# AlessioSam/LADiff

Hardware: AMD Instinct MI355X
Metric: motions/sec (196-frame, 50-step DDIM, bs128) (higher is better)
Workload: dtype f16x3+f32; 1 GPU; headline:ddim50_cfg7.5_b128_f196_c263_humanml3d; prompts_per_gpu=128, global_batch=128, frames=196, scheduler=ddim, denoising_steps=50, parallelism=dp1, loop=persistent pipeline kernel (16-row blocks x 86)

## Files before the change

### ladiff_amd/csrc/api.hip

```cpp
#include <algorithm>
#include <cstdlib>
#include <atomic>
#include <cstdio>
#include <cstdlib>
#include <cstring>
#include <vector>

#include "model.h"
#include "../../include/ladiff_hip_debug.h"

using namespace ladiff;

namespace {

inline hipStream_t S(ladiff_stream_t s) { return reinterpret_cast<hipStream_t>(s); }

template <class W>
bool load_weights(W& dst, const float* const* ptrs) {
    constexpr int n = sizeof(W) / sizeof(const float*);
    if (ptrs == nullptr) return false;
    for (int i = 0; i < n; ++i)
        if (ptrs[i] == nullptr) return false;
    std::memcpy(&dst, ptrs, sizeof(W));
    return true;
// ... 345 lines not shown
    g_handoff = tagged;
    return 0;
}

int ladiff_debug_set_mlp_variant(int v) {
#ifdef LADIFF_STAMPS
    LADIFF_CHECK_ARG((v >= 0 && v <= 3) || (v >= 11 && v <= 17) || (v >= 21 && v <= 26));
#else
    LADIFF_CHECK_ARG(v >= 0 && v <= 3);
#endif
    g_mlp_variant = v;
    return 0;
}

int ladiff_debug_set_decoder_fusion(int on) {
    LADIFF_CHECK_ARG(on >= 0 && on <= 126 && (on & 3) != 3 && (on & 48) != 48);
    g_dec_out_cross = (on & 64) ? 0 : 1;
    g_dec_fused_mlp = on & 3;
    g_dec_small_rows_path = (on & 4) ? 0 : 1;
    g_dec_final_split = (on & 8) ? 0 : 1;
    g_dec_fused_attn = (on & 16) ? 0 : (on & 32) ? 2 : 1;
    return 0;
}

int ladiff_debug_set_stage_plan(int v) {
    LADIFF_CHECK_ARG(v >= 0 && v <= 1);
    g_stage_plan = v;
    return 0;
}

int ladiff_debug_set_poll_pause(int mask, int len) {
// ... 445 lines not shown
    return 0;
}

int ladiff_vae_decode_graphed(void* graph, const float* const* w, const float* const* w_split, uint64_t weights_generation, const float* z,
                              const int32_t* lengths, const int32_t* counts, const int32_t* row_off, int total_rows, int B, int F, int T,
                              int C, float* feats, void* ws, size_t ws_bytes, ladiff_stream_t stream) {
    DecodeGraph* dg = reinterpret_cast<DecodeGraph*>(graph);
    DecoderW W, WS;
    LADIFF_CHECK_ARG(dg && load_weights(W, w) && z && lengths && feats && ws && B >= 0 && stream != nullptr);
    if (w_split != nullptr) LADIFF_CHECK_ARG(load_weights(WS, w_split));
    hipStream_t s = S(stream);
    const void* kp[7] = {z, lengths, counts, row_off, feats, ws, stream};
    const int ki[6] = {B, F, T, C, total_rows, w_split ? 1 : 0};
    uint64_t h = hash_ptrs(w, DEC_NPARAMS, 1469598103934665603ull);
    if (w_split) h = hash_ptrs(w_split, DEC_NPARAMS, h ^ 0x9e3779b97f4a7c15ull);
    h ^= (uint64_t)(g_dec_fused_mlp + 4 * g_dec_small_rows_path + 8 * g_dec_final_split + 16 * g_mlp_variant + 4096 * g_dec_fused_attn) * 0x100000001b3ull;
    const bool same = dg->exec && std::memcmp(kp, dg->key_ptrs, sizeof(kp)) == 0 && std::memcmp(ki, dg->key_ints, sizeof(ki)) == 0 &&
                      h == dg->key_hash && weights_generation == dg->key_gen &&
                      (dg->epoch == g_graph_epoch.load() || g_graph_epoch_rule.load() == 0);
    if (!same) {
        if (dg->exec) { LADIFF_HIP(hipStreamSynchronize(s)); (void)hipGraphExecDestroy(dg->exec); dg->exec = nullptr; }
        LADIFF_TRY(dec_mlp_prepare());
        LADIFF_TRY(dec_qkv_attn_prepare());
        LADIFF_TRY(dec_cross_prepare());
        hipGraph_t gr = nullptr;
        LADIFF_TRY(capture_stream(&dg->cap, &dg->cap_dev));
        const hipStream_t cs = dg->cap;
        LADIFF_HIP(hipStreamBeginCapture(cs, hipStreamCaptureModeThreadLocal));
        int rc = 0;
        if (row_off != nullptr) {
            rc = launch_zero_fill(feats, (size_t)B * F * C, cs);
        }
        if (rc == 0) rc = vae_decode(W, w_split ? &WS : nullptr, z, lengths, counts, row_off, total_rows, B, F, T, C, feats, (float*)ws,
                                     ws_bytes / sizeof(float), cs);
        const hipError_t ec = hipStreamEndCapture(cs, &gr);
        if (rc != 0) { if (gr) (void)hipGraphDestroy(gr); return rc; }
        LADIFF_HIP(ec);
        const hipError_t ei = hipGraphInstantiate(&dg->exec, gr, nullptr, nullptr, 0);
        ++g_graph_instantiations;
// ... 24 lines not shown
```

### ladiff_amd/csrc/attention.hip

```cpp
#include "kernels.h"

namespace ladiff {

constexpr int SA_FMAX = LADIFF_MAX_FRAMES;
constexpr int SA_NKT = SA_FMAX / 32;

struct AttnGeom { int nheads, ld, koff, voff, out_ld, causal; };

__global__ __launch_bounds__(256) void dec_self_attn_kernel(const float* __restrict__ qkv, const int32_t* __restrict__ lengths,
                                                            const uint32_t* __restrict__ keybits, float* __restrict__ out,
                                                            int B, int F, int split_out, const AttnGeom g,
                                                            const int32_t* __restrict__ row_off, int shared_qkv) {
    __shared__ __attribute__((aligned(16))) float Ks[SA_FMAX * DH];
    __shared__ __attribute__((aligned(16))) float Vs[SA_FMAX * DH];
    const int tid = threadIdx.x, lane = tid & 63, wave = tid >> 6;
    const int b = blockIdx.y / g.nheads, h = blockIdx.y % g.nheads;
    int len = F;
    uint32_t kb[SA_NKT + 1];
    if (keybits != nullptr) {
        len = 1;
#pragma unroll
        for (int i = 0; i < SA_NKT; ++i) {
            kb[i] = keybits[(size_t)b * 8 + i];
            if (kb[i]) len = 32 * i + 32 - __builtin_clz(kb[i]);
// ... 143 lines not shown
#pragma unroll
        for (int i = 0; i < NKT; ++i) {
            kb[i] = keybits[(size_t)b * 8 + i];
            if (kb[i]) len = 32 * i + 32 - __builtin_clz(kb[i]);
        }
        len = len > F ? F : len;
    } else {
        len = lengths != nullptr ? lengths[b] : F;
        len = len < 1 ? 1 : (len > F ? F : len);
#pragma unroll
        for (int i = 0; i < NKT; ++i) kb[i] = len >= 32 * i + 32 ? 0xFFFFFFFFu : (len > 32 * i ? (1u << (len - 32 * i)) - 1u : 0u);
    }
    const int nkt = (len + 31) >> 5;
    size_t row0 = (size_t)b * F;
    if (row_off != nullptr) { row0 = row_off[b]; F = row_off[b + 1] - row_off[b]; }
    const size_t base = (shared_qkv ? (size_t)0 : row0) * g.ld + h * DH;

    const int qt = wave;
    const int q = lane & 31, h2 = lane >> 5;
    const int qrow = qt * 32 + q;

    s16x8 qh[4], ql[4];
#pragma unroll
    for (int ks = 0; ks < 4; ++ks) {
        float v[8] = {0.f, 0.f, 0.f, 0.f, 0.f, 0.f, 0.f, 0.f};
        if (qrow < F) {
            const f32x4 a = ld4(qkv + base + (size_t)qrow * g.ld + 16 * ks + 8 * h2);
            const f32x4 c = ld4(qkv + base + (size_t)qrow * g.ld + 16 * ks + 8 * h2 + 4);
#pragma unroll
            for (int e = 0; e < 4; ++e) { v[e] = a[e] * (0.125f * 1.4426950408889634f); v[4 + e] = c[e] * (0.125f * 1.4426950408889634f); }
// ... 319 lines not shown
```

### ladiff_amd/csrc/dec_cross.hip

```cpp
#include <mutex>
#include "kernels.h"
#include "tile_mma.h"

namespace ladiff { extern unsigned long long* g_sys_stamps; }

namespace ladiff {

namespace {
constexpr int TM = LADIFF_MAX_LATENTS;
}

__global__ __launch_bounds__(256) void dec_cross_prep_kernel(const DecCrossPrepBatch pb, int B, int T, int tiles_per_wg) {
    const int h = blockIdx.y, layer = blockIdx.z, tid = threadIdx.x, lane = tid & 63, c16 = lane & 15, kq = lane >> 4;
    const int wave = __builtin_amdgcn_readfirstlane(tid >> 6);
    const float* __restrict__ kv = pb.kv[layer]; const float* __restrict__ wq = pb.wq[layer]; const float* __restrict__ bq = pb.bq[layer];
    const float* __restrict__ wo = pb.wo[layer]; float* __restrict__ gu = pb.gu[layer];
    float* __restrict__ cc = gu + (size_t)B * H * T * 2 * D;
    const int M = T * B, ntiles = (M + 15) / 16;
    float gq[4][16], uo[4][16], bqv[16];
#pragma unroll
    for (int t = 0; t < 4; ++t) {
        const int n = 64 * wave + 16 * t + c16;
#pragma unroll
        for (int s = 0; s < 16; ++s) gq[t][s] = wq[(size_t)(h * DH + 16 * kq + s) * D + n];
// ... 86 lines not shown
                const f32x4 u4 = ld4(up + 64 * k);
                acc[k][0] = fmaf(pj, u4[0], acc[k][0]); acc[k][1] = fmaf(pj, u4[1], acc[k][1]);
                acc[k][2] = fmaf(pj, u4[2], acc[k][2]); acc[k][3] = fmaf(pj, u4[3], acc[k][3]);
            }
        }
    }
}

template <int TT>
__global__ __launch_bounds__(256) void dec_cross_apply_kernel(const float* __restrict__ x, const float* __restrict__ gu,
                                                              const float* __restrict__ cc, const int32_t* __restrict__ counts,
                                                              const float* __restrict__ bo, const float* __restrict__ g2,
                                                              const float* __restrict__ b2, int F, int rows_per_wg,
                                                              float* __restrict__ y, float* __restrict__ ys,
                                                              const int32_t* __restrict__ row_off, const float* __restrict__ g1,
                                                              const float* __restrict__ b1) {
    extern __shared__ __attribute__((aligned(16))) float sm[];
    constexpr int T = TT, HT = H * TT;
    const int b = blockIdx.x, tid = threadIdx.x, lane = tid & 63, wave = tid >> 6;
    const float* src = gu + (size_t)b * HT * 2 * D;
    for (int u = tid; u < HT * 2 * D / 4; u += 256) st4(sm + 4 * u, ld4(src + 4 * u));
    float* cs = sm + (size_t)HT * 2 * D;
    if (tid < HT) cs[tid] = cc[(size_t)b * HT + tid];
    int nv = counts != nullptr ? counts[b] : T;
    nv = nv > T ? T : nv;
    __syncthreads();
    const int l16 = lane & 15, grp = lane >> 4, c0 = 4 * l16;
    f32x4 bo4[4], gg[4], bb[4];
#pragma unroll
    for (int k = 0; k < 4; ++k) { bo4[k] = ld4(bo + c0 + 64 * k); gg[k] = ld4(g2 + c0 + 64 * k); bb[k] = ld4(b2 + c0 + 64 * k); }
    size_t row0 = (size_t)b * F;
    if (row_off != nullptr) { row0 = row_off[b]; F = row_off[b + 1] - row_off[b]; }
    const int f0 = blockIdx.y * rows_per_wg;
    const int f1 = f0 + rows_per_wg < F ? f0 + rows_per_wg : F;
    for (int fb = f0; fb < f1; fb += 16) {
        const int f = fb + 4 * wave + grp;
        const bool live = f < f1;
        const size_t row = row0 + (live ? f : f1 - 1);
        f32x4 xv[4], acc[4];
#pragma unroll
        for (int k = 0; k < 4; ++k) xv[k] = ld4(x + row * D + c0 + 64 * k);
        if (g1 != nullptr) {
            float s1 = 0.f;
#pragma unroll
            for (int k = 0; k < 4; ++k) s1 += (xv[k][0] + xv[k][1]) + (xv[k][2] + xv[k][3]);
            const float mean1 = row16_sum(s1) * (1.f / 256.f);
            float q1 = 0.f;
#pragma unroll
            for (int k = 0; k < 4; ++k)
#pragma unroll
                for (int i = 0; i < 4; ++i) { const float dlt = xv[k][i] - mean1; q1 += dlt * dlt; }
            const float rstd1 = rsqrtf(row16_sum(q1) * (1.f / 256.f) + LN_EPS);
#pragma unroll
            for (int k = 0; k < 4; ++k) {
                const f32x4 ga = ld4(g1 + c0 + 64 * k), be = ld4(b1 + c0 + 64 * k);
#pragma unroll
// ... 348 lines not shown
}

int launch_decoder_cross_prep(const DecCrossPrepBatch& pb, int n, int B, int T, hipStream_t s) {
    if (B == 0 || n == 0) return 0;
    if (T < 1 || T > TM || n > DEC_PREP_MAX) return LADIFF_ERR_SHAPE;
    const int ntiles = (T * B + 15) / 16;
    int tpw = 1;
    while (tpw < 8 && (ntiles + 2 * tpw - 1) / (2 * tpw) * H * n >= 160) tpw *= 2;
    hipLaunchKernelGGL(dec_cross_prep_kernel, dim3((ntiles + tpw - 1) / tpw, H, n), dim3(256), 0, s, pb, B, T, tpw);
    LADIFF_LAUNCH_CHECK();
    return 0;
}

int launch_decoder_cross_apply(const float* x, const float* bo, const float* g2, const float* b2, const int32_t* counts, int B, int F,
                               int T, const float* gu_ws, float* y, float* ys, hipStream_t s, const int32_t* row_off, const float* g1,
                               const float* b1) {
    if (B == 0 || F == 0) return 0;
    if (T < 1 || T > TM) return LADIFF_ERR_SHAPE;
    const float* gu = gu_ws;
    const float* cc = gu_ws + (size_t)B * H * T * 2 * D;
    int chunks = (512 + B - 1) / B;
    if (chunks < 1) chunks = 1;
    if (chunks > (F + 3) / 4) chunks = (F + 3) / 4;
    const int rows_per_wg = ((F + chunks - 1) / chunks + 15) / 16 * 16;
    chunks = (F + rows_per_wg - 1) / rows_per_wg;
    const size_t lds = ((size_t)H * T * 2 * D + H * T) * sizeof(float);
    LADIFF_TRY(dec_cross_prepare());
#define LADIFF_DC_CASE(TT)                                                                                                   \
    case TT:                                                                                                                 \
        hipLaunchKernelGGL(dec_cross_apply_kernel<TT>, dim3(B, chunks), dim3(256), lds, s, x, gu, cc, counts, bo, g2, b2, F, \
                           rows_per_wg, y, ys, row_off, g1, b1);                                                                              \
        break;
    switch (T) {
        LADIFF_DC_CASE(1) LADIFF_DC_CASE(2) LADIFF_DC_CASE(3) LADIFF_DC_CASE(4)
        LADIFF_DC_CASE(5) LADIFF_DC_CASE(6) LADIFF_DC_CASE(7) LADIFF_DC_CASE(8)
        default: return LADIFF_ERR_SHAPE;
    }
#undef LADIFF_DC_CASE
    LADIFF_LAUNCH_CHECK();
    return 0;
}

int launch_decoder_out_cross(const float* att_s, const float* x0, const float* wo_s, const float* bo, const float* g1, const float* b1,
                             const float* bo_c, const float* g2, const float* b2, const int32_t* counts, int B, int F, int T,
                             const float* gu_ws, float* y, float* ys, hipStream_t s, const int32_t* row_off) {
    if (B == 0 || F == 0) return 0;
// ... 25 lines not shown
```

### ladiff_amd/csrc/decoder.hip

```cpp
#include "model.h"
#ifdef LADIFF_STAMPS
#include <cstdlib>
#endif

namespace ladiff {

#ifdef LADIFF_STAMPS
#define DEC_CUT() do { if (dec_cut >= 0 && ++dec_launched >= dec_cut) return 0; } while (0)
#else
#define DEC_CUT() do { } while (0)
#endif

constexpr int DEC_SMALL_ROWS = 4096;
std::atomic<int> g_dec_out_cross{1};
std::atomic<int> g_dec_fused_attn{1};
std::atomic<int> g_dec_final_split{1};
std::atomic<int> g_dec_small_rows_path{1};
std::atomic<int> g_dec_fused_mlp{1};

static GemmArgs lin(const float* A, int lda, const float* W, const float* bias, float* Y, int ldy, int M, int N, int K,
                    int act = ACT_NONE) {
    GemmArgs g;
    g.A = A; g.lda = lda; g.W = W; g.ldw = K; g.bias = bias; g.Y = Y; g.ldy = ldy; g.M = M; g.N = N; g.K = K; g.act = act;
    return g;
}

size_t dec_ws_floats(int B, size_t rows, int T) {
    return rows * (16 * D + 3 * D + D + FF) + (rows + 63) / 64 * 64 + (size_t)NL * ((size_t)T * B * 2 * D + dec_cross_ws_floats(B, T)) +
           (size_t)LADIFF_MAX_FRAMES * (2 * D + 3 * D);
}

int vae_decode(const DecoderW& w, const DecoderW* wsp, const float* z, const int32_t* lengths, const int32_t* counts,
               const int32_t* row_off, int R, int B, int F, int T, int C, float* feats, float* ws, size_t ws_floats, hipStream_t s) {
// ... 16 lines not shown
    for (int i = 0; i < 4; ++i) { P[i] = p; p += MD; }
    for (int i = 0; i < NSKIP; ++i) { SK[i] = p; p += MD; }
    for (int i = 0; i < 4; ++i) { Ps[i] = sp ? p : nullptr; p += MD; }
    for (int i = 0; i < NSKIP; ++i) { SKs[i] = sp ? p : nullptr; p += MD; }
    float* qkv = p; p += 3 * MD;
    float* att = p; p += MD;
    float* hid = p; p += (size_t)M * FF;
    float* kv = p; p += (size_t)NL * T * B * 2 * D;
    float* guws = p; p += (size_t)NL * dec_cross_ws_floats(B, T);
    int32_t* row_out = reinterpret_cast<int32_t*>(p); p += ((size_t)M + 63) / 64 * 64;
    float* pex = p; p += (size_t)LADIFF_MAX_FRAMES * D;
    float* pexs = p; p += (size_t)LADIFF_MAX_FRAMES * D;
    float* qkv0 = p;
    const size_t kv_l = (size_t)T * B * 2 * D, gu_l = dec_cross_ws_floats(B, T);

    {
        GemmArgs g[NL];
        DecCrossPrepBatch pb;
        for (int l = 0; l < NL; ++l) {
            const DecLayerW& L = w.layer[l];
            g[l] = lin(z, D, L.cross_attn.in_w + (size_t)D * D, L.cross_attn.in_b + D, kv + l * kv_l, 2 * D, T * B, 2 * D, D);
            pb.kv[l] = kv + l * kv_l; pb.wq[l] = L.cross_attn.in_w; pb.bq[l] = L.cross_attn.in_b; pb.wo[l] = L.cross_attn.out_w;
            pb.gu[l] = guws + l * gu_l;
        }
        LADIFF_TRY(launch_gemm_batch(g, NL, s)); DEC_CUT();
        LADIFF_TRY(launch_decoder_cross_prep(pb, NL, B, T, s)); DEC_CUT();
    }

    const bool small = sp && M < DEC_SMALL_ROWS && g_dec_small_rows_path;
    const bool fused_attn = sp && g_dec_fused_attn && (M >= DEC_SMALL_ROWS || g_dec_fused_attn == 2);
    auto krs = [&](const float* A, int K, const float* W, const float* bias, float* Y, float* Ys, int ldy, int N, int act,
                   const float* res, int rows) -> int {
        KrArgs g;
        g.A = A; g.lda = K; g.W = W; g.ldw = K; g.bias = bias; g.Y = Y; g.Ys = Ys; g.ldy = ldy; g.M = rows; g.N = N; g.K = K; g.act = act;
        g.res = res; g.ldres = D; g.split = 1;
        return launch_gemm_kr(g, s);
    };

    auto gemm_ln = [&](const float* A, int K, const float* W, const float* Wsp, const float* bias, const float* res,
                       const NormW& n1, const NormW* n2, float* dst, float* dsts) -> int {
        GemmArgs g = lin(A, K, sp ? Wsp : W, bias, dst, D, M, D, K);
        g.res = res; g.ldres = D;
        if (!sp) {
            g.ln_g = n1.g; g.ln_b = n1.b;
            if (n2) { g.ln2_g = n2->g; g.ln2_b = n2->b; }
            return launch_gemm(g, s);
        }
        g.split = 1;
        LADIFF_TRY(launch_gemm(g, s));
        if (n2)
            return launch_reduce_rows(dst, 1, M, nullptr, nullptr, RED_LN, n1.g, n1.b, nullptr, 0, nullptr, nullptr, 1, 1, 0,
                                      0, dst, dsts, s, nullptr, n2->g, n2->b);
        return launch_reduce_rows(dst, 1, M, nullptr, nullptr, RED_LN, n1.g, n1.b, nullptr, 0, nullptr, nullptr, 1, 1, 0, 0,
                                  dst, dsts, s);
    };

    if (ragged) { LADIFF_TRY(launch_broadcast_pe_ragged(w.query_pe, row_off, B, F, F, P[0], Ps[0], row_out, s)); DEC_CUT(); }
    else { LADIFF_TRY(launch_broadcast_pe(w.query_pe, B, F, P[0], Ps[0], s)); DEC_CUT(); }
    const float* cur = P[0]; const float* curs = Ps[0];
    for (int l = 0; l < NL; ++l) {
        const DecLayerW& L = w.layer[l];
        const DecLayerW& Ls = sp ? wsp->layer[l] : w.layer[l];
        const bool is_in = l < NSKIP, is_out = l > NSKIP, last = l == NL - 1;
        if (is_out) {
            const LinearW& sk = w.skip[l - NSKIP - 1];
            if (small) {
                RowLnArgs g;
                g.A = curs; g.lda = D; g.A2 = SKs[NL - 1 - l]; g.lda2 = D; g.K1 = D; g.W = wsp->skip[l - NSKIP - 1].w; g.ldw = 2 * D; g.bias = sk.b;
                g.Y = P[3]; g.Ys = Ps[3]; g.ldy = D; g.M = M; g.K = 2 * D;
                LADIFF_TRY(launch_gemm_rowln(g, s)); DEC_CUT();
            } else {
            GemmArgs g = lin(sp ? curs : cur, D, sp ? wsp->skip[l - NSKIP - 1].w : sk.w, sk.b, P[3], D, M, D, 2 * D);
            g.A2 = sp ? SKs[NL - 1 - l] : SK[NL - 1 - l]; g.lda2 = D; g.K1 = D;
// ... 7 lines not shown
            LADIFF_TRY(launch_broadcast_pe(w.query_pe, 1, F, pex, sp ? pexs : nullptr, s)); DEC_CUT();
            if (small) { LADIFF_TRY(krs(pexs, D, Ls.self_attn.in_w, L.self_attn.in_b, qkv0, nullptr, 3 * D, 3 * D, ACT_NONE, nullptr, F)); DEC_CUT(); }
            else {
            GemmArgs g = lin(sp ? pexs : pex, D, Ls.self_attn.in_w, L.self_attn.in_b, qkv0, 3 * D, F, 3 * D, D);
            g.split = sp ? 1 : 0;
            LADIFF_TRY(launch_gemm(g, s)); DEC_CUT();
            }
        } else if (fused_attn) {
        } else if (small) {
            LADIFF_TRY(krs(curs, D, Ls.self_attn.in_w, L.self_attn.in_b, qkv, nullptr, 3 * D, 3 * D, ACT_NONE, nullptr, M)); DEC_CUT();
        } else {
            GemmArgs g = lin(sp ? curs : cur, D, Ls.self_attn.in_w, L.self_attn.in_b, qkv, 3 * D, M, 3 * D, D);
            g.split = sp ? 1 : 0;
            LADIFF_TRY(launch_gemm(g, s)); DEC_CUT();
        }
        const float* qkv_l = shared ? qkv0 : qkv;
        if (fused_attn && !shared) { LADIFF_TRY(launch_dec_qkv_attn(curs, Ls.self_attn.in_w, L.self_attn.in_b, lengths, row_off, att, B, F, 1, s)); DEC_CUT(); }
        else if (sp) { LADIFF_TRY(launch_self_attention_split(qkv_l, lengths, nullptr, att, B, F, H, 0, 1, s, row_off, shared)); DEC_CUT(); }
        else { LADIFF_TRY(launch_decoder_self_attention(qkv_l, lengths, nullptr, att, B, F, 0, s, row_off, shared)); DEC_CUT(); }
        const NormW* n1_late = nullptr;
        if (sp && !small && g_dec_out_cross) {
            LADIFF_TRY(launch_decoder_out_cross(att, cur, Ls.self_attn.out_w, L.self_attn.out_b, L.norm1.g, L.norm1.b, L.cross_attn.out_b,
                                                L.norm2.g, L.norm2.b, counts, B, F, T, guws + l * gu_l, P[2], Ps[2], s, row_off)); DEC_CUT();
        } else {
        if (sp) {
            if (small) { LADIFF_TRY(krs(att, D, Ls.self_attn.out_w, L.self_attn.out_b, P[1], nullptr, D, D, ACT_NONE, cur, M)); DEC_CUT(); }
            else {
            GemmArgs g = lin(att, D, Ls.self_attn.out_w, L.self_attn.out_b, P[1], D, M, D, D);
            g.res = cur; g.ldres = D; g.split = 1;
            LADIFF_TRY(launch_gemm(g, s)); DEC_CUT();
            }
            n1_late = &L.norm1;
        } else {
            LADIFF_TRY(gemm_ln(att, D, L.self_attn.out_w, Ls.self_attn.out_w, L.self_attn.out_b, cur, L.norm1, nullptr, P[1], nullptr)); DEC_CUT();
        }
        LADIFF_TRY(launch_decoder_cross_apply(P[1], L.cross_attn.out_b, L.norm2.g, L.norm2.b, counts, B, F, T, guws + l * gu_l, P[2],
                                              Ps[2], s, row_off, n1_late ? n1_late->g : nullptr, n1_late ? n1_late->b : nullptr)); DEC_CUT();
        }
        float* dst = is_in ? SK[l] : P[0];
        float* dsts = is_in ? SKs[l] : Ps[0];
        if (sp && g_dec_fused_mlp && (M >= dec_mlp_min_rows() || g_dec_fused_mlp == 2)) {
            LADIFF_TRY(launch_dec_mlp(Ps[2], P[2], Ls.lin1.w, L.lin1.b, Ls.lin2.w, L.lin2.b, L.norm3.g, L.norm3.b,
                                      last ? w.norm.g : nullptr, last ? w.norm.b : nullptr, dst, dsts, M, s)); DEC_CUT();
        } else if (small) {
            LADIFF_TRY(krs(Ps[2], D, Ls.lin1.w, L.lin1.b, nullptr, hid, FF, FF, ACT_GELU, nullptr, M)); DEC_CUT();
            LADIFF_TRY(krs(hid, FF, Ls.lin2.w, nullptr, qkv, nullptr, D, D, ACT_NONE, nullptr, M)); DEC_CUT();
            LADIFF_TRY(launch_reduce_rows(qkv, 4, M, L.lin2.b, P[2], RED_LN, L.norm3.g, L.norm3.b, nullptr, 0, nullptr, nullptr, 1, 1, 0, 0,
                                          dst, dsts, s, nullptr, last ? w.norm.g : nullptr, last ? w.norm.b : nullptr));
        } else {
            GemmArgs g = lin(sp ? Ps[2] : P[2], D, Ls.lin1.w, L.lin1.b, sp ? nullptr : hid, FF, M, FF, D, ACT_GELU);
            g.split = sp ? 1 : 0; if (sp) g.Ys = hid;
            LADIFF_TRY(launch_gemm(g, s)); DEC_CUT();
// ... 22 lines not shown
```

### ladiff_amd/csrc/gemm_kr.h

```cpp
#pragma once
#include "common.h"

namespace ladiff {

struct KrArgs {
    const float* A = nullptr;  int lda = 0;
    const float* A2 = nullptr; int lda2 = 0;
    int K1 = 0;
    const float* W = nullptr;  int ldw = 0;
    const float* bias = nullptr;
    float* Y = nullptr;        int ldy = 0;
    float* Ys = nullptr;
    int split = 0;
    int M = 0, N = 0, K = 0;
    int act = ACT_NONE;
    const float* res = nullptr; int ldres = 0;
    unsigned long long* stamps = nullptr;
};

int launch_gemm_kr(const KrArgs& a, hipStream_t s);

struct RowLnArgs {
    const float* A = nullptr;  int lda = 0;
    const float* A2 = nullptr; int lda2 = 0; int K1 = 0;
    const float* W = nullptr;  int ldw = 0;
    const float* bias = nullptr;
    const float* res = nullptr; int ldres = 0;
    const float* ln_g = nullptr; const float* ln_b = nullptr;
    float* Y = nullptr; float* Ys = nullptr; int ldy = 0;
    int M = 0, K = 0;
};
int launch_gemm_rowln(const RowLnArgs& a, hipStream_t s);

struct CombineGemmArgs {
    const float* P = nullptr; size_t plane = 0; int S = 0;
    const float* bias2 = nullptr;
    const float* ln_g = nullptr; const float* ln_b = nullptr;
    const float* tab = nullptr; int tab_step_stride = 0; const int32_t* d_step = nullptr;
    const float* W = nullptr; int ldw = 0;
    const float* bias = nullptr;
    const float* res = nullptr; int ldres = 0;
    float* Y = nullptr; float* Ys = nullptr; int ldy = 0;
    int M = 0;
};
int launch_combine_gemm(const CombineGemmArgs& a, hipStream_t s);
// ... 3 lines not shown
```

### ladiff_amd/csrc/gemm_rowln.hip

```cpp
#include "gemm_kr.h"

namespace ladiff {

namespace {
template <int N> __device__ __forceinline__ void wait_vm() { asm volatile("s_waitcnt vmcnt(%0)" ::"n"(N) : "memory"); }
__device__ __forceinline__ void dma16(const float* g, float* l) {
    __builtin_amdgcn_global_load_lds(g, (__attribute__((address_space(3))) void*)l, 16, 0, 0);
}
}

__global__ __launch_bounds__(512) void gemm_rowln_kernel(const RowLnArgs p) {
    constexpr int BM = 16, BN = 256;
    constexpr int ROWS = BM + BN;
    constexpr int STAGE = ROWS * 64;
    constexpr int PCS = ROWS / 4;
    constexpr int PPW = PCS / 4;
    constexpr int RN = 4;
    constexpr int CLD = BN + 4;
    static_assert(2 * PPW <= 63, "vmcnt is 6 bits");

    __shared__ __attribute__((aligned(1024))) float lds[2 * STAGE];

    const int tid = threadIdx.x, lane = tid & 63;
    const int wave = __builtin_amdgcn_readfirstlane(tid >> 6);
    const int argM = pin_s(p.M), nk = pin_s(p.K) >> 6;
    const int row0 = blockIdx.x * BM;

    if (wave >= 4) {
        const int pw = wave - 4;
        const int rl = 4 * pw + (lane >> 4);
        const int kl = ((lane & 15) ^ rl) << 2;
        const float* const argA = pin_s(p.A); const float* const argW = pin_s(p.W);
        const int lda = pin_s(p.lda), ldw = pin_s(p.ldw);
        int gr = row0 + rl; gr = gr < argM ? gr : argM - 1;
        const float* const arow = argA + (size_t)gr * lda + kl;
        const int K1 = pin_s(p.K1);
        const float* const arow2 = p.A2 != nullptr ? p.A2 + (size_t)gr * p.lda2 + kl - K1 : arow;
        const float* const wrow = argW + (size_t)rl * ldw + kl;
        float* const lbase = lds + 4 * pw * 64;
        auto issue = [&](int kt) __attribute__((always_inline)) {
            float* const dst = lbase + (kt & 1) * STAGE;
// ... 13 lines not shown
        return;
    }

    float* const argY = pin_s(p.Y); float* const argYs = pin_s(p.Ys);
    const float* const argRes = pin_s(p.res);
    const int ldres = pin_s(p.ldres), ldy = pin_s(p.ldy);
    const int c = lane * 4;
    const f32x4 zero = {0.f, 0.f, 0.f, 0.f};
    const f32x4 bi = p.bias != nullptr ? ld4(p.bias + c) : zero;
    const bool ln = p.ln_g != nullptr;
    const f32x4 gg = ln ? ld4(p.ln_g + c) : zero, bb = ln ? ld4(p.ln_b + c) : zero;
    f32x4 rv[4];
#pragma unroll
    for (int e = 0; e < 4; ++e) {
        const int gr = row0 + 4 * wave + e;
        rv[e] = (argRes != nullptr && gr < argM) ? ld4g(argRes + (size_t)gr * ldres + c) : zero;
    }

    f32x4 acc[RN];
#pragma unroll
    for (int j = 0; j < RN; ++j) acc[j] = zero;
    const int frow = lane & 15, fk = lane >> 4;
    for (int kt = 0; kt < nk; ++kt) {
        const float* sa = lds + (kt & 1) * STAGE;
        const float* sb = sa + (BM + 64 * wave) * 64;
        __builtin_amdgcn_s_barrier();
        s16x8 ah[2], al[2], bh[2][RN], bl[2][RN];
#pragma unroll
        for (int g = 0; g < 2; ++g) {
            const int ch = 4 * g + fk, cl = 8 + 4 * g + fk;
            ah[g] = __builtin_bit_cast(s16x8, ld4(sa + frow * 64 + ((ch ^ frow) << 2)));
// ... 235 lines not shown
```

### ladiff_amd/csrc/kernels.h

```cpp
#pragma once
#include "common.h"
#include "noise_gen.h"

namespace ladiff {

enum RedMode : int { RED_PLAIN = 0, RED_LN = 1, RED_LN_ADD = 2, RED_LN_MOD = 3 };
int launch_reduce_rows(const float* P, int S, int M, const float* bias, const float* res, int mode, const float* g,
                       const float* b, const float* tab, int tab_step_stride, const int32_t* d_step,
                       const int32_t* counts, int Bs, int T, int pad_row, int b_off, float* out, float* outs, hipStream_t s,
                       const int32_t* d_base = nullptr, const float* g2 = nullptr, const float* b2 = nullptr);
int launch_split_rows(const float* x, float* y, int R, int K, hipStream_t s);
int launch_gather_rows(const float* src, const int32_t* index, int n_rows, int row_floats, float* dst, hipStream_t s);
int launch_split_range_stats(const float* const* xs, const int64_t* counts, int n, int64_t max_count, unsigned long long* stats,
                             hipStream_t s);
int launch_layernorm(const float* x, const float* g, const float* b, float* y, int M, hipStream_t s);
constexpr int DEC_PREP_MAX = 9;
struct DecCrossPrepBatch { const float* kv[DEC_PREP_MAX]; const float* wq[DEC_PREP_MAX]; const float* bq[DEC_PREP_MAX];
                           const float* wo[DEC_PREP_MAX]; float* gu[DEC_PREP_MAX]; };
constexpr int ROW_BATCH_MAX = 9;
struct RowBatch { const float* a[ROW_BATCH_MAX]; const float* g[ROW_BATCH_MAX]; const float* b[ROW_BATCH_MAX]; float* y[ROW_BATCH_MAX]; };
int launch_layernorm_batch(const RowBatch& rb, int n, int M, hipStream_t s);
int launch_ca_table_input_batch(const RowBatch& rb, int n_layers, int step_stride, int n, int B2, hipStream_t s, int split_out = 0);
int launch_ca_table_input(const float* nval, const float* beta, const float* mod, int step_stride, int n, int B2, float* u,
                          hipStream_t s);
int launch_add_pe(const float* sample, const float* pe, int Bs, int b_off, int b_n, int T, float* x, float* xs, hipStream_t s);
int launch_broadcast_pe(const float* pe, int B, int F, float* x, float* xs, hipStream_t s);
int launch_broadcast_pe_ragged(const float* pe, const int32_t* row_off, int B, int F, int F_out, float* x, float* xs, int32_t* row_out,
                               hipStream_t s);
int launch_relu(const float* x, float* y, size_t n, hipStream_t s);
int launch_pad_rows(const float* src, const float* srcb, float* dst, float* dstb, int C, int Np, hipStream_t s);
int launch_zero_fill(float* x, size_t n, hipStream_t s);
int launch_silu(const float* x, float* y, size_t n, hipStream_t s);
int launch_sinusoid(const int64_t* t, int n, float* out, hipStream_t s);
int launch_cfg_step(const float* eps, float* lat, const float* coef, const int32_t* d_step, const float* noise,
                    float g, int cfg, int B, int T, hipStream_t s);
int launch_advance(int32_t* d_step, hipStream_t s);
int launch_step_tail(float* x, float* xs, const float* ng, const float* nb, float* lat, const float* coef, int32_t* d_step,
                     const float* noise, const float* pe, float g, int cfg, int B, int T, hipStream_t s, const NoiseGen& gen = NoiseGen{0u, 0u, 0u, 0});
int launch_noise_fill(const NoiseGen& gen, int step0, int n, int B, int T, float* out, hipStream_t s);
int launch_init_latents(const float* noise, const int32_t* counts, float sigma, float* lat, int B, int T, hipStream_t s);
int launch_finalize_latents(const float* lat, const int32_t* counts, float* z, int B, int T, hipStream_t s, const unsigned* status = nullptr);

int launch_dec_qkv_attn(const float* xs, const float* w, const float* bias, const int32_t* lengths, const int32_t* row_off, float* out,
// ... 9 lines not shown
int launch_lca_kv(const float* key, const float* value, int B, int N, float* att, hipStream_t s);
int launch_lca_apply(const float* q, const float* att, const int32_t* counts, int Bs, int b_off, int b_n, int T, const float* mod,
                     int step_stride, int sample_stride, const int32_t* d_step, const float* g, const float* be, float* u,
                     hipStream_t s);
int launch_denoiser_self_attention_general(const float* qkv, const float* text_kv, int N, const float* tables, int kv_off,
                                           int step_stride, const int32_t* d_step, const int32_t* counts, int Bs, int b_off,
                                           int b_n, int T, float* out, hipStream_t s);

size_t dec_cross_ws_floats(int B, int T);
int launch_decoder_cross_prep(const DecCrossPrepBatch& pb, int n, int B, int T, hipStream_t s);
int launch_decoder_out_cross(const float* att_s, const float* x0, const float* wo_s, const float* bo, const float* g1, const float* b1,
                             const float* bo_c, const float* g2, const float* b2, const int32_t* counts, int B, int F, int T,
                             const float* gu_ws, float* y, float* ys, hipStream_t s, const int32_t* row_off);
int launch_decoder_cross_apply(const float* x, const float* bo, const float* g2, const float* b2, const int32_t* counts, int B, int F,
                               int T, const float* gu_ws, float* y, float* ys, hipStream_t s, const int32_t* row_off = nullptr,
                               const float* g1 = nullptr, const float* b1 = nullptr);

int launch_feats2joints(const float* feats, const float* mean, const float* stdv, int B, int F, int C, int J, float* joints,
                        hipStream_t s);

int launch_denoiser_self_attention(const float* qkv, const float* text_kv, const float* tables, int kv_off,
                                   int step_stride, const int32_t* d_step, const int32_t* counts, int Bs, int b_off,
                                   int b_n, int T, float* out, int split_out, hipStream_t s);
int launch_decoder_self_attention(const float* qkv, const int32_t* lengths, const uint32_t* keybits, float* out, int B, int F,
                                  int split_out, hipStream_t s, const int32_t* row_off = nullptr, int shared_qkv = 0);
int launch_self_attention(const float* qkv, const int32_t* lengths, const uint32_t* keybits, float* out, int B, int F, int nheads,
                          int causal, int split_out, hipStream_t s, const int32_t* row_off = nullptr);
int launch_self_attention_split(const float* qkv, const int32_t* lengths, const uint32_t* keybits, float* out, int B, int F,
                                 int nheads, int causal, int split_out, hipStream_t s, const int32_t* row_off = nullptr, int shared_qkv = 0);
int launch_decoder_cross_attention(const float* q, const float* kv, const int32_t* counts, float* out, int B, int F,
                                   int T, int split_out, hipStream_t s);
// ... 3 lines not shown
```

### ladiff_amd/csrc/model.h

```cpp
#pragma once
#include <atomic>
#include "gemm.h"
#include "gemm_kr.h"
#include "kernels.h"
#include "weights.h"

namespace ladiff {

constexpr int DEN_OFF_CA_MOD = 0;
constexpr int DEN_OFF_FFN_MOD = 2 * D;
constexpr int DEN_OFF_TIME_KV = 4 * D;
constexpr int DEN_LAYER_STRIDE = 6 * D;
constexpr int DEN_STEP_STRIDE = NL * DEN_LAYER_STRIDE;

size_t den_tables_floats(int n_steps);
size_t den_text_cache_floats(int B2, int n_steps, int ntxt = 1);
size_t den_text_ws_floats(int B2, int n_steps, int ntxt = 1);
size_t den_forward_ws_floats(int B2, int T);
int denoiser_time_tables(const DenoiserW& w, const float* sinus, int n, float* tables, float* ws, size_t ws_floats, hipStream_t s);
int denoiser_text_cache(const DenoiserW& w, const float* text, int B2, const float* tables, int n_steps, float* cache,
                        float* ws, size_t ws_floats, hipStream_t s, int ntxt = 1);
int denoiser_forward(const DenoiserW& w, const DenoiserW* w_split, const float* tables, const int32_t* d_step,
                     const float* cache, int n_steps, const float* sample, int Bs, int dup, int T, const int32_t* counts, float* eps, float* ws,
                     size_t ws_floats, hipStream_t s, int b_lo = 0, int b_n = -1, int loop_mode = 0, int ntxt = 1,
                     const int32_t* d_base = nullptr);
const float* den_cache_tkv(const float* cache, int B2, int ntxt);
const float* den_cache_ctab(const float* cache, int B2, int ntxt);
int denoiser_text_static(const DenoiserW& w, const float* text, int B2, float* cache, float* ws, size_t ws_floats, hipStream_t s);
int denoiser_ctab(const DenoiserW& w, const float* tables_lo, int n, float* cache, int B2, float* u, size_t u_floats, hipStream_t s,
                  const DenoiserW* w_split = nullptr);
int linear_cross_attention(const DenoiserW& w, int layer, const float* x, const float* xf, const float* emb, const int32_t* counts,
                           int B, int T, int N, float* out, float* ws, size_t ws_floats, hipStream_t s);
size_t linear_cross_attention_ws_floats(int B, int T, int N);
void den_loop_io(float* ws, int rows, float** x, float** xs);

extern std::atomic<int> g_dec_fused_mlp;
extern std::atomic<int> g_dec_small_rows_path;
extern std::atomic<int> g_dec_final_split;
extern std::atomic<int> g_dec_out_cross;
extern std::atomic<int> g_stage_plan;
extern std::atomic<int> g_poll_pause;
extern std::atomic<int> g_stage_delay;
extern std::atomic<int> g_pace;
extern std::atomic<int> g_look_ahead_from, g_small_upto;
extern std::atomic<int> g_dec_fused_attn;
extern std::atomic<int> g_mlp_variant;
int dec_mlp_prepare();
int dec_qkv_attn_prepare();
int dec_cross_prepare();
int dec_mlp_min_rows();
size_t dec_ws_floats(int B, size_t rows, int T);
int vae_decode(const DecoderW& w, const DecoderW* w_split, const float* z, const int32_t* lengths, const int32_t* counts,
               const int32_t* row_off, int R, int B, int F, int T, int C, float* feats, float* ws, size_t ws_floats, hipStream_t s);

int launch_dec_mlp(const float* xs, const float* x, const float* w1, const float* b1, const float* w2, const float* b2, const float* g3,
                   const float* be3, const float* g4, const float* be4, float* y, float* ys, int M, hipStream_t s);

size_t enc_ws_floats(int B, int F, int T, int C);
int vae_encode(const EncoderW& w, const EncoderW* w_split, const float* features, const int32_t* lengths,
               const int32_t* counts, const float* eps, int B, int F, int T, int C, float* mu, float* sd, float* latent, float* ws,
               size_t ws_floats, hipStream_t s);

#ifdef LADIFF_STAMPS
extern unsigned long long* g_sys_stamps;
// ... 42 lines not shown
```

### ladiff_amd/csrc/rowops.hip

```cpp
#include <algorithm>

#include "kernels.h"

namespace ladiff {

constexpr int ROWS_PER_BLOCK = 4;

__device__ __forceinline__ void row_stats(const f32x4 v, float& mean, float& rstd) {
    float s = wave_sum(v[0] + v[1] + v[2] + v[3]);
    mean = s * (1.f / 256.f);
    float q = 0.f;
#pragma unroll
    for (int i = 0; i < 4; ++i) { const float d = v[i] - mean; q += d * d; }
    q = wave_sum(q);
    rstd = rsqrtf(q * (1.f / 256.f) + LN_EPS);
}

__global__ __launch_bounds__(256) void layernorm_kernel(const float* __restrict__ x, const float* __restrict__ g,
                                                        const float* __restrict__ b, float* __restrict__ y, int M) {
    const int row = blockIdx.x * ROWS_PER_BLOCK + (threadIdx.x >> 6);
    const int c = (threadIdx.x & 63) * 4;
    if (row >= M) return;
    f32x4 v = ld4(x + (size_t)row * D + c);
    float mean, rstd;
// ... 189 lines not shown
    const int c = (threadIdx.x & 63) * 4;
    if (row >= M) return;
    const f32x4 v = ld4(pe + (size_t)(row % F) * D + c);
    st4(x + (size_t)row * D + c, v);
    if (xs != nullptr) store_split4(xs + (size_t)row * D, c, v);
}

__global__ __launch_bounds__(256) void broadcast_pe_ragged_kernel(const float* __restrict__ pe, const int32_t* __restrict__ row_off,
                                                                  int F, int F_out, float* __restrict__ x, float* __restrict__ xs,
                                                                  int32_t* __restrict__ row_out) {
    const int b = blockIdx.y, f = blockIdx.x * ROWS_PER_BLOCK + (threadIdx.x >> 6);
    const int c = (threadIdx.x & 63) * 4;
    const int r0 = row_off[b];
    if (f >= F || f >= row_off[b + 1] - r0) return;
    const size_t row = (size_t)r0 + f;
    const f32x4 v = ld4(pe + (size_t)f * D + c);
    st4(x + row * D + c, v);
    if (xs != nullptr) store_split4(xs + row * D, c, v);
    if (c == 0) row_out[row] = b * F_out + f;
}
int launch_broadcast_pe_ragged(const float* pe, const int32_t* row_off, int B, int F, int F_out, float* x, float* xs, int32_t* row_out,
                               hipStream_t s) {
    if (B == 0) return 0;
    hipLaunchKernelGGL(broadcast_pe_ragged_kernel, dim3((F + ROWS_PER_BLOCK - 1) / ROWS_PER_BLOCK, B), dim3(256), 0, s, pe, row_off, F,
                       F_out, x, xs, row_out);
    LADIFF_LAUNCH_CHECK();
    return 0;
}

int launch_broadcast_pe(const float* pe, int B, int F, float* x, float* xs, hipStream_t s) {
    const int M = B * F;
    hipLaunchKernelGGL(broadcast_pe_kernel, dim3((M + ROWS_PER_BLOCK - 1) / ROWS_PER_BLOCK), dim3(256), 0, s, pe, F, M, x, xs);
    LADIFF_LAUNCH_CHECK();
    return 0;
}

__global__ __launch_bounds__(256) void gather_rows_kernel(const float* __restrict__ src, const int32_t* __restrict__ index, int n_rows,
                                                          int row4, float* __restrict__ dst) {
    const int row = blockIdx.x * ROWS_PER_BLOCK + (threadIdx.x >> 6);
    if (row >= n_rows) return;
// ... 420 lines not shown
```

Baseline: 11390 motions/s.

## Dedupe decoder layer-0 self-attention by unique length and overlap cross prep on side stream

New measurement: 11400 motions/s, median of 2. About the same (+0.0%).

```diff
diff --git a/ladiff_amd/csrc/api.hip b/ladiff_amd/csrc/api.hip
--- a/ladiff_amd/csrc/api.hip
+++ b/ladiff_amd/csrc/api.hip
@@ -383,7 +383,8 @@
 }
 
 int ladiff_debug_set_decoder_fusion(int on) {
-    LADIFF_CHECK_ARG(on >= 0 && on <= 126 && (on & 3) != 3 && (on & 48) != 48);
+    LADIFF_CHECK_ARG(on >= 0 && on <= 254 && (on & 3) != 3 && (on & 48) != 48);
+    g_dec_layer0_table = (on & 128) ? 0 : 1;
     g_dec_out_cross = (on & 64) ? 0 : 1;
     g_dec_fused_mlp = on & 3;
     g_dec_small_rows_path = (on & 4) ? 0 : 1;
@@ -859,7 +860,8 @@
     const int ki[6] = {B, F, T, C, total_rows, w_split ? 1 : 0};
     uint64_t h = hash_ptrs(w, DEC_NPARAMS, 1469598103934665603ull);
     if (w_split) h = hash_ptrs(w_split, DEC_NPARAMS, h ^ 0x9e3779b97f4a7c15ull);
-    h ^= (uint64_t)(g_dec_fused_mlp + 4 * g_dec_small_rows_path + 8 * g_dec_final_split + 16 * g_mlp_variant + 4096 * g_dec_fused_attn) * 0x100000001b3ull;
+    h ^= (uint64_t)(g_dec_fused_mlp + 4 * g_dec_small_rows_path + 8 * g_dec_final_split + 16 * g_mlp_variant + 4096 * g_dec_fused_attn + 16384 * g_dec_out_cross +
+                    32768 * g_dec_layer0_table) * 0x100000001b3ull;
     const bool same = dg->exec && std::memcmp(kp, dg->key_ptrs, sizeof(kp)) == 0 && std::memcmp(ki, dg->key_ints, sizeof(ki)) == 0 &&
                       h == dg->key_hash && weights_generation == dg->key_gen &&
                       (dg->epoch == g_graph_epoch.load() || g_graph_epoch_rule.load() == 0);
@@ -868,6 +870,7 @@
         LADIFF_TRY(dec_mlp_prepare());
         LADIFF_TRY(dec_qkv_attn_prepare());
         LADIFF_TRY(dec_cross_prepare());
+        LADIFF_TRY(dec_front_prepare());
         hipGraph_t gr = nullptr;
         LADIFF_TRY(capture_stream(&dg->cap, &dg->cap_dev));
         const hipStream_t cs = dg->cap;
diff --git a/ladiff_amd/csrc/attention.hip b/ladiff_amd/csrc/attention.hip
--- a/ladiff_amd/csrc/attention.hip
+++ b/ladiff_amd/csrc/attention.hip
@@ -181,6 +181,7 @@
     const int nkt = (len + 31) >> 5;
     size_t row0 = (size_t)b * F;
     if (row_off != nullptr) { row0 = row_off[b]; F = row_off[b + 1] - row_off[b]; }
+    if (F <= 0) return;
     const size_t base = (shared_qkv ? (size_t)0 : row0) * g.ld + h * DH;
 
     const int qt = wave;
diff --git a/ladiff_amd/csrc/dec_cross.hip b/ladiff_amd/csrc/dec_cross.hip
--- a/ladiff_amd/csrc/dec_cross.hip
+++ b/ladiff_amd/csrc/dec_cross.hip
@@ -124,7 +124,8 @@
                                                               const float* __restrict__ b2, int F, int rows_per_wg,
                                                               float* __restrict__ y, float* __restrict__ ys,
                                                               const int32_t* __restrict__ row_off, const float* __restrict__ g1,
-                                                              const float* __restrict__ b1) {
+                                                              const float* __restrict__ b1, const int32_t* __restrict__ tab_off,
+                                                              const int32_t* __restrict__ len_idx) {
     extern __shared__ __attribute__((aligned(16))) float sm[];
     constexpr int T = TT, HT = H * TT;
     const int b = blockIdx.x, tid = threadIdx.x, lane = tid & 63, wave = tid >> 6;
@@ -143,13 +144,28 @@
     if (row_off != nullptr) { row0 = row_off[b]; F = row_off[b + 1] - row_off[b]; }
     const int f0 = blockIdx.y * rows_per_wg;
     const int f1 = f0 + rows_per_wg < F ? f0 + rows_per_wg : F;
+    size_t trow0 = 0;
+    int tlen = F;
+    if (tab_off != nullptr) { const int u = len_idx[b]; trow0 = tab_off[u]; tlen = tab_off[u + 1] - tab_off[u]; }
     for (int fb = f0; fb < f1; fb += 16) {
         const int f = fb + 4 * wave + grp;
         const bool live = f < f1;
         const size_t row = row0 + (live ? f : f1 - 1);
+        if (tab_off != nullptr && f >= tlen) {
+            if (live) {
+                const f32x4 z4 = {0.f, 0.f, 0.f, 0.f};
+#pragma unroll
+                for (int k = 0; k < 4; ++k) {
+                    st4(y + row * D + c0 + 64 * k, z4);
+                    if (ys != nullptr) store_split4(ys + row * D, c0 + 64 * k, z4);
+                }
+            }
+            continue;
+        }
+        const size_t xrow = tab_off != nullptr ? trow0 + f : row;
         f32x4 xv[4], acc[4];
 #pragma unroll
-        for (int k = 0; k < 4; ++k) xv[k] = ld4(x + row * D + c0 + 64 * k);
+        for (int k = 0; k < 4; ++k) xv[k] = ld4(x + xrow * D + c0 + 64 * k);
         if (g1 != nullptr) {
             float s1 = 0.f;
 #pragma unroll
@@ -528,7 +544,8 @@
 
 int launch_decoder_cross_apply(const float* x, const float* bo, const float* g2, const float* b2, const int32_t* counts, int B, int F,
                                int T, const float* gu_ws, float* y, float* ys, hipStream_t s, const int32_t* row_off, const float* g1,
-                               const float* b1) {
+                               const float* b1, const int32_t* tab_off, const int32_t* len_idx) {
+    if ((tab_off == nullptr) != (len_idx == nullptr)) return LADIFF_ERR_ARG;
     if (B == 0 || F == 0) return 0;
     if (T < 1 || T > TM) return LADIFF_ERR_SHAPE;
     const float* gu = gu_ws;
@@ -543,7 +560,7 @@
 #define LADIFF_DC_CASE(TT)                                                                                                   \
     case TT:                                                                                                                 \
         hipLaunchKernelGGL(dec_cross_apply_kernel<TT>, dim3(B, chunks), dim3(256), lds, s, x, gu, cc, counts, bo, g2, b2, F, \
-                           rows_per_wg, y, ys, row_off, g1, b1);                                                                              \
+                           rows_per_wg, y, ys, row_off, g1, b1, tab_off, len_idx);                                                                          \
         break;
     switch (T) {
         LADIFF_DC_CASE(1) LADIFF_DC_CASE(2) LADIFF_DC_CASE(3) LADIFF_DC_CASE(4)
diff --git a/ladiff_amd/csrc/decoder.hip b/ladiff_amd/csrc/decoder.hip
--- a/ladiff_amd/csrc/decoder.hip
+++ b/ladiff_amd/csrc/decoder.hip
@@ -1,4 +1,6 @@
 #include "model.h"
+#include <mutex>
+#include <vector>
 #ifdef LADIFF_STAMPS
 #include <cstdlib>
 #endif
@@ -17,6 +19,50 @@
 std::atomic<int> g_dec_final_split{1};
 std::atomic<int> g_dec_small_rows_path{1};
 std::atomic<int> g_dec_fused_mlp{1};
+
+std::atomic<int> g_dec_layer0_table{1};
+
+namespace {
+struct FrontSet { int dev; bool busy; hipStream_t side; hipEvent_t fork, join; };
+std::mutex g_front_mu;
+std::vector<FrontSet*> g_front_sets;
+FrontSet* front_acquire() {
+    int dev = 0;
+    if (hipGetDevice(&dev) != hipSuccess) return nullptr;
+    std::lock_guard<std::mutex> lock(g_front_mu);
+    for (FrontSet* f : g_front_sets) if (f->dev == dev && !f->busy) { f->busy = true; return f; }
+    FrontSet* f = new FrontSet{dev, true, nullptr, nullptr, nullptr};
+    if (hipStreamCreateWithFlags(&f->side, hipStreamNonBlocking) != hipSuccess ||
+        hipEventCreateWithFlags(&f->fork, hipEventDisableTiming) != hipSuccess ||
+        hipEventCreateWithFlags(&f->join, hipEventDisableTiming) != hipSuccess) {
+        if (f->fork) (void)hipEventDestroy(f->fork);
+        if (f->side) (void)hipStreamDestroy(f->side);
+        delete f;
+        return nullptr;
+    }
+    g_front_sets.push_back(f);
+    return f;
+}
+void front_release(FrontSet* f) { std::lock_guard<std::mutex> lock(g_front_mu); f->busy = false; }
+struct FrontHold {
+    FrontSet* f = nullptr;
+    hipStream_t s = nullptr;
+    bool forked = false;
+    int join() {
+        if (!forked) return 0;
+        forked = false;
+        return (int)hipStreamWaitEvent(s, f->join, 0);
+    }
+    ~FrontHold() { if (f) { (void)join(); front_release(f); } }
+};
+}
+
+int dec_front_prepare() {
+    FrontSet* f = front_acquire();
+    if (f == nullptr) return (int)hipErrorOutOfMemory;
+    front_release(f);
+    return 0;
+}
 
 static GemmArgs lin(const float* A, int lda, const float* W, const float* bias, float* Y, int ldy, int M, int N, int K,
                     int act = ACT_NONE) {
@@ -63,7 +109,20 @@
     float* qkv0 = p;
     const size_t kv_l = (size_t)T * B * 2 * D, gu_l = dec_cross_ws_floats(B, T);
 
+    const bool small = sp && M < DEC_SMALL_ROWS && g_dec_small_rows_path;
+    const int U = B < LADIFF_MAX_FRAMES ? B : LADIFF_MAX_FRAMES;
+    const bool l0tab = sp && g_dec_layer0_table && (size_t)2 * U + 1 + B + M <= 3 * MD;
+    FrontHold front;
+    if (l0tab && !small) {
+        front.f = front_acquire();
+        if (front.f == nullptr) return (int)hipErrorOutOfMemory;
+        front.s = s;
+        LADIFF_HIP(hipEventRecord(front.f->fork, s));
+        LADIFF_HIP(hipStreamWaitEvent(front.f->side, front.f->fork, 0));
+        front.forked = true;
+    }
     {
+        const hipStream_t zs = front.f ? front.f->side : s;
         GemmArgs g[NL];
         DecCrossPrepBatch pb;
         for (int l = 0; l < NL; ++l) {
@@ -72,11 +131,13 @@
             pb.kv[l] = kv + l * kv_l; pb.wq[l] = L.cross_attn.in_w; pb.bq[l] = L.cross_attn.in_b; pb.wo[l] = L.cross_attn.out_w;
             pb.gu[l] = guws + l * gu_l;
         }
-        LADIFF_TRY(launch_gemm_batch(g, NL, s)); DEC_CUT();
-        LADIFF_TRY(launch_decoder_cross_prep(pb, NL, B, T, s)); DEC_CUT();
-    }
-
-    const bool small = sp && M < DEC_SMALL_ROWS && g_dec_small_rows_path;
+        int rc = launch_gemm_batch(g, NL, zs);
+        if (rc == 0) rc = launch_decoder_cross_prep(pb, NL, B, T, zs);
+        if (front.f) { const hipError_t e = hipEventRecord(front.f->join, zs); if (rc == 0) rc = (int)e; }
+        if (rc != 0) return rc;
+        DEC_CUT(); DEC_CUT();
+    }
+
     const bool fused_attn = sp && g_dec_fused_attn && (M >= DEC_SMALL_ROWS || g_dec_fused_attn == 2);
     auto krs = [&](const float* A, int K, const float* W, const float* bias, float* Y, float* Ys, int ldy, int N, int act,
                    const float* res, int rows) -> int {
@@ -104,8 +165,14 @@
                                   dst, dsts, s);
     };
 
-    if (ragged) { LADIFF_TRY(launch_broadcast_pe_ragged(w.query_pe, row_off, B, F, F, P[0], Ps[0], row_out, s)); DEC_CUT(); }
-    else { LADIFF_TRY(launch_broadcast_pe(w.query_pe, B, F, P[0], Ps[0], s)); DEC_CUT(); }
+    if (ragged) { LADIFF_TRY(launch_broadcast_pe_ragged(w.query_pe, row_off, B, F, F, l0tab ? nullptr : P[0], l0tab ? nullptr : Ps[0], row_out, s)); DEC_CUT(); }
+    else if (!l0tab) { LADIFF_TRY(launch_broadcast_pe(w.query_pe, B, F, P[0], Ps[0], s)); DEC_CUT(); }
+    int32_t* tab_len = reinterpret_cast<int32_t*>(qkv);
+    int32_t* tab_off = tab_len + U;
+    int32_t* len_idx = tab_off + U + 1;
+    int32_t* tab_f = len_idx + B;
+    float* att_tab = att;
+    float* n1tab = hid;
     const float* cur = P[0]; const float* curs = Ps[0];
     for (int l = 0; l < NL; ++l) {
         const DecLayerW& L = w.layer[l];
@@ -143,6 +210,17 @@
             g.split = sp ? 1 : 0;
             LADIFF_TRY(launch_gemm(g, s)); DEC_CUT();
         }
+        if (shared && l0tab) {
+            LADIFF_TRY(launch_dec_len_table(lengths, row_off, B, F, U, tab_len, tab_off, len_idx, tab_f, s)); DEC_CUT();
+            LADIFF_TRY(launch_self_attention_split(qkv0, tab_len, nullptr, att_tab, U, F, H, 0, 1, s, tab_off, 1)); DEC_CUT();
+            RowLnArgs g;
+            g.A = att_tab; g.lda = D; g.K1 = D; g.W = Ls.self_attn.out_w; g.ldw = D; g.bias = L.self_attn.out_b; g.res = pex; g.ldres = D;
+            g.res_map = tab_f; g.ln_g = L.norm1.g; g.ln_b = L.norm1.b; g.Y = n1tab; g.ldy = D; g.M = M; g.K = D; g.d_M = tab_off + U;
+            LADIFF_TRY(launch_gemm_rowln(g, s)); DEC_CUT();
+            LADIFF_TRY(front.join());
+            LADIFF_TRY(launch_decoder_cross_apply(n1tab, L.cross_attn.out_b, L.norm2.g, L.norm2.b, counts, B, F, T, guws + l * gu_l, P[2],
+                                                  Ps[2], s, row_off, nullptr, nullptr, tab_off, len_idx)); DEC_CUT();
+        } else {
         const float* qkv_l = shared ? qkv0 : qkv;
         if (fused_attn && !shared) { LADIFF_TRY(launch_dec_qkv_attn(curs, Ls.self_attn.in_w, L.self_attn.in_b, lengths, row_off, att, B, F, 1, s)); DEC_CUT(); }
         else if (sp) { LADIFF_TRY(launch_self_attention_split(qkv_l, lengths, nullptr, att, B, F, H, 0, 1, s, row_off, shared)); DEC_CUT(); }
@@ -165,6 +243,7 @@
         }
         LADIFF_TRY(launch_decoder_cross_apply(P[1], L.cross_attn.out_b, L.norm2.g, L.norm2.b, counts, B, F, T, guws + l * gu_l, P[2],
                                               Ps[2], s, row_off, n1_late ? n1_late->g : nullptr, n1_late ? n1_late->b : nullptr)); DEC_CUT();
+        }
         }
         float* dst = is_in ? SK[l] : P[0];
         float* dsts = is_in ? SKs[l] : Ps[0];
diff --git a/ladiff_amd/csrc/gemm_kr.h b/ladiff_amd/csrc/gemm_kr.h
--- a/ladiff_amd/csrc/gemm_kr.h
+++ b/ladiff_amd/csrc/gemm_kr.h
@@ -29,6 +29,8 @@
     const float* ln_g = nullptr; const float* ln_b = nullptr;
     float* Y = nullptr; float* Ys = nullptr; int ldy = 0;
     int M = 0, K = 0;
+    const int32_t* d_M = nullptr;
+    const int32_t* res_map = nullptr;
 };
 int launch_gemm_rowln(const RowLnArgs& a, hipStream_t s);
 
diff --git a/ladiff_amd/csrc/gemm_rowln.hip b/ladiff_amd/csrc/gemm_rowln.hip
--- a/ladiff_amd/csrc/gemm_rowln.hip
+++ b/ladiff_amd/csrc/gemm_rowln.hip
@@ -23,8 +23,12 @@
 
     const int tid = threadIdx.x, lane = tid & 63;
     const int wave = __builtin_amdgcn_readfirstlane(tid >> 6);
-    const int argM = pin_s(p.M), nk = pin_s(p.K) >> 6;
+    const int nk = pin_s(p.K) >> 6;
     const int row0 = blockIdx.x * BM;
+    int argM_ = p.M;
+    if (p.d_M != nullptr) { const int m = __builtin_amdgcn_readfirstlane(*p.d_M); argM_ = m < argM_ ? m : argM_; }
+    const int argM = pin_s(argM_);
+    if (row0 >= argM) return;
 
     if (wave >= 4) {
         const int pw = wave - 4;
@@ -68,7 +72,7 @@
 #pragma unroll
     for (int e = 0; e < 4; ++e) {
         const int gr = row0 + 4 * wave + e;
-        rv[e] = (argRes != nullptr && gr < argM) ? ld4g(argRes + (size_t)gr * ldres + c) : zero;
+        rv[e] = (argRes != nullptr && gr < argM) ? ld4g(argRes + (size_t)(p.res_map != nullptr ? p.res_map[gr] : gr) * ldres + c) : zero;
     }
 
     f32x4 acc[RN];
diff --git a/ladiff_amd/csrc/kernels.h b/ladiff_amd/csrc/kernels.h
--- a/ladiff_amd/csrc/kernels.h
+++ b/ladiff_amd/csrc/kernels.h
@@ -27,6 +27,8 @@
 int launch_broadcast_pe(const float* pe, int B, int F, float* x, float* xs, hipStream_t s);
 int launch_broadcast_pe_ragged(const float* pe, const int32_t* row_off, int B, int F, int F_out, float* x, float* xs, int32_t* row_out,
                                hipStream_t s);
+int launch_dec_len_table(const int32_t* lengths, const int32_t* row_off, int B, int F, int U, int32_t* tab_len, int32_t* tab_off,
+                         int32_t* len_idx, int32_t* tab_f, hipStream_t s);
 int launch_relu(const float* x, float* y, size_t n, hipStream_t s);
 int launch_pad_rows(const float* src, const float* srcb, float* dst, float* dstb, int C, int Np, hipStream_t s);
 int launch_zero_fill(float* x, size_t n, hipStream_t s);
@@ -66,7 +68,8 @@
                              const float* gu_ws, float* y, float* ys, hipStream_t s, const int32_t* row_off);
 int launch_decoder_cross_apply(const float* x, const float* bo, const float* g2, const float* b2, const int32_t* counts, int B, int F,
                                int T, const float* gu_ws, float* y, float* ys, hipStream_t s, const int32_t* row_off = nullptr,
-                               const float* g1 = nullptr, const float* b1 = nullptr);
+                               const float* g1 = nullptr, const float* b1 = nullptr, const int32_t* tab_off = nullptr,
+                               const int32_t* len_idx = nullptr);
 
 int launch_feats2joints(const float* feats, const float* mean, const float* stdv, int B, int F, int C, int J, float* joints,
                         hipStream_t s);
diff --git a/ladiff_amd/csrc/model.h b/ladiff_amd/csrc/model.h
--- a/ladiff_amd/csrc/model.h
+++ b/ladiff_amd/csrc/model.h
@@ -38,6 +38,7 @@
 extern std::atomic<int> g_dec_small_rows_path;
 extern std::atomic<int> g_dec_final_split;
 extern std::atomic<int> g_dec_out_cross;
+extern std::atomic<int> g_dec_layer0_table;
 extern std::atomic<int> g_stage_plan;
 extern std::atomic<int> g_poll_pause;
 extern std::atomic<int> g_stage_delay;
@@ -48,6 +49,7 @@
 int dec_mlp_prepare();
 int dec_qkv_attn_prepare();
 int dec_cross_prepare();
+int dec_front_prepare();
 int dec_mlp_min_rows();
 size_t dec_ws_floats(int B, size_t rows, int T);
 int vae_decode(const DecoderW& w, const DecoderW* w_split, const float* z, const int32_t* lengths, const int32_t* counts,
diff --git a/ladiff_amd/csrc/rowops.hip b/ladiff_amd/csrc/rowops.hip
--- a/ladiff_amd/csrc/rowops.hip
+++ b/ladiff_amd/csrc/rowops.hip
@@ -227,9 +227,11 @@
     const int r0 = row_off[b];
     if (f >= F || f >= row_off[b + 1] - r0) return;
     const size_t row = (size_t)r0 + f;
-    const f32x4 v = ld4(pe + (size_t)f * D + c);
-    st4(x + row * D + c, v);
-    if (xs != nullptr) store_split4(xs + row * D, c, v);
+    if (x != nullptr) {
+        const f32x4 v = ld4(pe + (size_t)f * D + c);
+        st4(x + row * D + c, v);
+        if (xs != nullptr) store_split4(xs + row * D, c, v);
+    }
     if (c == 0) row_out[row] = b * F_out + f;
 }
 int launch_broadcast_pe_ragged(const float* pe, const int32_t* row_off, int B, int F, int F_out, float* x, float* xs, int32_t* row_out,
@@ -237,6 +239,49 @@
     if (B == 0) return 0;
     hipLaunchKernelGGL(broadcast_pe_ragged_kernel, dim3((F + ROWS_PER_BLOCK - 1) / ROWS_PER_BLOCK, B), dim3(256), 0, s, pe, row_off, F,
                        F_out, x, xs, row_out);
+    LADIFF_LAUNCH_CHECK();
+    return 0;
+}
+
+__global__ __launch_bounds__(256) void dec_len_table_kernel(const int32_t* __restrict__ lengths, const int32_t* __restrict__ row_off, int B,
+                                                            int F, int U, int32_t* __restrict__ tab_len, int32_t* __restrict__ tab_off,
+                                                            int32_t* __restrict__ len_idx, int32_t* __restrict__ tab_f) {
+    static_assert(LADIFF_MAX_FRAMES + 2 <= 256, "a thread per length, one more for the totals");
+    __shared__ int present[256], slot[256], offs[256];
+    __shared__ unsigned long long mask[4];
+    const int v = threadIdx.x;
+    auto length_of = [&](int b) {
+        int e = row_off != nullptr ? row_off[b + 1] - row_off[b] : (lengths[b] < 1 ? 1 : lengths[b]);
+        e = e > F ? F : e;
+        return e < 0 ? 0 : e;
+    };
+    present[v] = 0;
+    __syncthreads();
+    for (int b = v; b < B; b += 256) { const int e = length_of(b); if (e > 0) present[e] = 1; }
+    __syncthreads();
+    const unsigned long long mine = __ballot(present[v] != 0);
+    if ((v & 63) == 0) mask[v >> 6] = mine;
+    __syncthreads();
+    int rank = 0, off = 0;
+    for (int q = 0; q < 4; ++q) {
+        unsigned long long m = mask[q];
+        if (64 * q + 63 >= v) m &= v > 64 * q ? (1ull << (v - 64 * q)) - 1ull : 0ull;
+        while (m) { const int w = 64 * q + __builtin_ctzll(m); ++rank; off += w; m &= m - 1; }
+    }
+    slot[v] = rank; offs[v] = off;
+    if (v >= 1 && v <= F && present[v] && rank < U) { tab_len[rank] = v; tab_off[rank] = off; }
+    __syncthreads();
+    const int nu = slot[F + 1], total = offs[F + 1];
+    if (v >= nu && v < U) { tab_len[v] = 0; tab_off[v] = total; }
+    if (v == 0) tab_off[U] = total;
+    for (int b = v; b < B; b += 256) { const int e = length_of(b); len_idx[b] = e > 0 ? slot[e] : 0; }
+    for (int q = 0; q < 4; ++q)
+        for (unsigned long long m = mask[q]; m; m &= m - 1) { const int w = 64 * q + __builtin_ctzll(m); if (v < w) tab_f[offs[w] + v] = v; }
+}
+int launch_dec_len_table(const int32_t* lengths, const int32_t* row_off, int B, int F, int U, int32_t* tab_len, int32_t* tab_off,
+                         int32_t* len_idx, int32_t* tab_f, hipStream_t s) {
+    if (B < 1 || F < 1 || F > LADIFF_MAX_FRAMES || U < 1 || U > LADIFF_MAX_FRAMES) return LADIFF_ERR_SHAPE;
+    hipLaunchKernelGGL(dec_len_table_kernel, dim3(1), dim3(256), 0, s, lengths, row_off, B, F, U, tab_len, tab_off, len_idx, tab_f);
     LADIFF_LAUNCH_CHECK();
     return 0;
 }
```
